# YaqiangCao/cLoops

Measured on AMD Instinct MI355X. Metric: PETs clustered/sec (whole node) + wall-clock for mode-3 eps x minPts sweep, higher is better.
Workload: dtype int32; 1 GPU; synthetic-200M-23chr-mode3 (BASELINE.json configs[3]); variant=cDBSCAN2, pets=200000000, chromosomes=23, chained_cut=True, final_cut=3871, candidate_loops=3651369, parallelism=23 chromosomes LPT-sharded over 1 GPU(s)

## Files before the change

cloops_amd/csrc/k_lists.hip:

```cpp
#include "cl_chrom.h"

#ifdef CLOOPS_DEVEL
#define L_ABL(bit) (g.dbg2 & (bit))
#else
#define L_ABL(bit) 0
#endif
#ifdef CLOOPS_DEVEL
__device__ unsigned long long g_lstat[32];
__device__ __forceinline__ void lstat_add(int slot, int v)
{
    int t = v;
    for (int o = 32; o > 0; o >>= 1) t += __shfl_down(t, o);
    if ((threadIdx.x & 63) == 0 && t) atomicAdd(&g_lstat[slot], (unsigned long long)t);
}
extern "C" void cl_debug_lstats(unsigned long long* out)
{
    (void)hipDeviceSynchronize();
    (void)hipMemcpyFromSymbol(out, HIP_SYMBOL(g_lstat), sizeof(g_lstat));
    unsigned long long z[32] = {0};
    (void)hipMemcpyToSymbol(HIP_SYMBOL(g_lstat), z, sizeof(z));
}
#define LSTAT_ON (g.dbg2 & (1 << 30))
#define LSTAT(slot, v) do { if (LSTAT_ON) lstat_add((slot), (v)); } while (0)
#else
// ... 476 lines not shown
        cgv[u] = cgloc[gidx]; wgv[u] = wgloc[gidx];
        const int b = t0 + u * 256 + (int)threadIdx.x;
        q[u] = b < npos ? bq[b] : 0; sp[u] = b < npos ? bsp[b] : 0;
    }
    {
        int2 fx[8];
#pragma unroll
        for (int u = 0; u < 8; ++u) {
            const int b = t0 + u * 256 + (int)threadIdx.x;
            const bool isc = (cbv[u] >> lane) & 1ull, isw = (wbv[u] >> lane) & 1ull;
            const int* wsrc = (BAND && q[u] < bandq) ? band : words;
            aux[u] = L_ABL(1 << 25) ? b : (isw ? wsrc[b] : (isc ? (V2 ? bkey[b] : (int)brow[b]) : 0));
            fx[u] = make_int2(INT_MIN, 0);
            if (V2 && CUT && !L_ABL(1 << 26)) {
                const unsigned long long anyb = cbv[u] | wbv[u];
                const int st = isc ? (sp[u] >> g.rbits) : 0;
                if (anyb) {
                    const int s_lo = __builtin_amdgcn_readlane(sp[u], __ffsll((long long)anyb) - 1) >> g.rbits;
                    const int s_hi = __builtin_amdgcn_readlane(sp[u], 63 - __clzll((long long)anyb)) >> g.rbits;
                    const int2 fa = fix[s_lo], fz = fix[s_hi];
                    if (isc) fx[u] = st == s_lo ? fa : (st == s_hi ? fz : fix[st]);
                }
            }
        }
#pragma unroll
        for (int u = 0; u < 8; ++u) {
            const int b = t0 + u * 256 + (int)threadIdx.x;
            const bool isw = (wbv[u] >> lane) & 1ull;
            if (V2 && CUT && b < fx[u].x) aux[u] = fx[u].y;
            if (isw) aux[u] = (int)lh_pack(aux[u], 0, 0);
        }
    }
    int cbase, wbase;
    {
        const int sb = blk >> 4;
        int pc = 0, pw_ = 0;
        for (int k = threadIdx.x; k < sb; k += 256) { const unsigned long long v = sup[k]; pc += (int)(unsigned)v; pw_ += (int)(unsigned)(v >> 32); }
        if (threadIdx.x < 16) { const int k = sb * 16 + (int)threadIdx.x; if (k < blk) { pc += bsum[k]; pw_ += bsum[nblk + 1 + k]; } }
#pragma unroll
        for (int o = 32; o > 0; o >>= 1) { pc += __shfl_down(pc, o); pw_ += __shfl_down(pw_, o); }
        if (lane == 0) { l_red[0][wv] = pc; l_red[1][wv] = pw_; }
        __syncthreads();
        cbase = l_red[0][0] + l_red[0][1] + l_red[0][2] + l_red[0][3];
        wbase = l_red[1][0] + l_red[1][1] + l_red[1][2] + l_red[1][3];
    }
    if (blk == nblk - 1 && threadIdx.x == 0) {
        const int C = cbase + bsum[blk], W = wbase + bsum[nblk + 1 + blk];
        lcnt[0] = C; lcnt[1] = W;
        cgrank[nblk * LG] = C; wgrank[nblk * LG] = W;
#ifdef CLOOPS_DEVEL
        if (LSTAT_ON) { atomicAdd(&g_lstat[8], (unsigned long long)C); atomicAdd(&g_lstat[9], (unsigned long long)W); atomicAdd(&g_lstat[11], 1ull); }
#endif
    }
#pragma unroll
    for (int u = 0; u < 8; ++u) {
        cgv[u] += cbase; wgv[u] += wbase;
        if (lane == 0) { const int gidx = (t0 >> 6) + u * 4 + wv; cgrank[gidx] = cgv[u]; wgrank[gidx] = wgv[u]; }
    }
#pragma unroll
    for (int u = 0; u < 8; ++u) {
        const int b = t0 + u * 256 + (int)threadIdx.x;
        const unsigned long long cb = cbv[u], wb = wbv[u];
        const bool isc = (cb >> lane) & 1ull, isw = (wb >> lane) & 1ull;
        if (L_ABL(1 << 27)) { if (q[u] + sp[u] + aux[u] == 0x7f123457) ckey[0] = 1; continue; }
        if (isc) {
            const int dst = cgv[u] + __popcll(cb & low_mask(lane));
            cpair[dst] = make_int2(q[u], sp[u]); ckey[dst] = aux[u];
            if (cpos) cpos[dst] = b;
            if (parent) parent[dst] = dst;
        } else if (isw) {
            const int dst = wgv[u] + __popcll(wb & low_mask(lane));
            wpair[dst] = make_int2(q[u], sp[u]); wpos[dst] = b; wenc[dst] = aux[u];
        }
    }
}

#define CH_PER 4
__global__ void __launch_bounds__(256)
k_chain_c(GridParams g, const int* __restrict__ lcnt, const int2* __restrict__ cpair, int* __restrict__ chainid,
          int* __restrict__ parent, int* __restrict__ compkey, int* __restrict__ ncore, int* __restrict__ bsize,
          int* __restrict__ usize, int* __restrict__ state, int* __restrict__ cskip,
          const int* __restrict__ strip_start, const unsigned long long* __restrict__ cmask, const int* __restrict__ cgrank,
          int* __restrict__ cstrip, int* __restrict__ sup, int nsup2, int* __restrict__ ckey_prune )
{
    const int C = lcnt[0];
    const int lane = threadIdx.x & 63;
    const int nmask = ~(g.peps - 1);
    {
        const int M = strip_start[g.S];
        for (int u = blockIdx.x * 256 + (int)threadIdx.x; u <= g.S + 1; u += gridDim.x * 256) {
            const int p = u <= g.S ? strip_start[u] : M;
            cstrip[u] = p < M ? core_rank(cmask, cgrank, p) : C;
        }
        if (blockIdx.x == 0) for (int k = threadIdx.x; k < nsup2; k += 256) sup[k] = 0;
    }
    int2 me[CH_PER], pv[CH_PER], nx[CH_PER];
#pragma unroll
    for (int e = 0; e < CH_PER; ++e) {
        const int c = (blockIdx.x * CH_PER + e) * 256 + (int)threadIdx.x;
        const bool in = c < C;
        me[e] = in ? cpair[c] : make_int2(0, 0);
        pv[e] = (in && c > 0) ? cpair[c - 1] : make_int2(0, INT_MIN);
        nx[e] = (in && c + 1 < C) ? cpair[c + 1] : make_int2(0, INT_MIN);
    }
#pragma unroll
    for (int e = 0; e < CH_PER; ++e) {
        const int c = (blockIdx.x * CH_PER + e) * 256 + (int)threadIdx.x;
        const bool in = c < C;
        const int p0 = me[e].y & nmask;
        const bool open = in && (c == 0 || (pv[e].y & nmask) != p0 || pv[e].x < me[e].x - g.eps);
        const bool last = in && (c + 1 >= C || (nx[e].y & nmask) != p0 || nx[e].x > me[e].x + g.eps);
        const unsigned long long ob = __ballot(open);
        const unsigned long long lb = __ballot(last) & (~0ull << lane);
        const int skip = (c - lane) + (lb ? __ffsll((long long)lb) : 64);
        const unsigned long long upto = ob & ((2ull << lane) - 1ull);
        int head = upto ? (c - lane) + 63 - __clzll((long long)upto) : -1;
        if (__any(in && !upto)) {
            int found = -1;
            for (int k0 = (c - lane) - 64; found < 0 && k0 >= 0; k0 -= 64) {
                const int j = k0 + lane;
                const int2 a = cpair[j];
                const int2 b = j > 0 ? cpair[j - 1] : make_int2(0, INT_MIN);
                const bool o = j == 0 || (b.y & nmask) != (a.y & nmask) || b.x < a.x - g.eps;
                const unsigned long long bal = __ballot(o);
                if (bal) found = k0 + 63 - __clzll((long long)bal);
            }
            if (!upto) head = found;
        }
        if (in) {
            chainid[c] = head;
            if (head == c) { parent[c] = c; compkey[c] = INT_MAX; ncore[c] = 0; bsize[c] = 0; usize[c] = 0; state[c] = ST_LIVE; }
            cskip[c] = skip;
            if (ckey_prune && c > 0 && (pv[e].y & nmask) == p0 && div_eps(g, pv[e].x) == div_eps(g, me[e].x)) ckey_prune[c] = INT_MAX;
        }
    }
}

#define LU_MAXB 4
__device__ __forceinline__ int lower_bound_pairs(const int2* __restrict__ pv, int lo, int hi, int val)
{
    while (hi - lo > 4) {
        const int qq = (hi - lo) >> 2;
        const int m1 = lo + qq, m2 = m1 + qq, m3 = m2 + qq;
        const int v1 = pv[m1].x, v2 = pv[m2].x, v3 = pv[m3].x;
        if (v1 >= val) hi = m1;
        else if (v2 >= val) { lo = m1 + 1; hi = m2; }
        else if (v3 >= val) { lo = m2 + 1; hi = m3; }
        else lo = m3 + 1;
    }
    while (lo < hi && pv[lo].x < val) ++lo;
    return lo;
}

struct HeadReset { int* compkey; int* ncore; int* bsize; int* usize; int* state; };
template <int NT, int HALO, bool FUSE>
__global__ void __launch_bounds__(256)
k_union_c(GridParams g, int ntiles, const int* __restrict__ lcnt, const int2* __restrict__ cpair, int* chainid,
          const int* __restrict__ cstrip, int* cskip, int* parent, HeadReset hr, int* __restrict__ ckey_prune ,
          int* __restrict__ ovlist, int* __restrict__ counters)
{
    constexpr int WIN = NT + HALO;
    constexpr int NCH = WIN / 64;
    __shared__ int2 lw[WIN];
    __shared__ int lx[WIN];
    __shared__ int lend[WIN];
    __shared__ unsigned long long l_ob[FUSE ? NCH : 1];
    __shared__ int l_found;
    const int C = lcnt[0];
    const int tile = ltile_of_block(blockIdx.x);
    const int t0 = tile * NT;
    if (tile >= ntiles || t0 >= C) return;
    const int base = t0 - HALO;
    const int lane = threadIdx.x & 63;
    const int nmask = ~(g.peps - 1);
    if (FUSE && threadIdx.x == 0) l_found = -1;
    int pf_tb[NT / 256], pf_b[NT / 256];
    {
        constexpr int SU = (WIN + 255) / 256;
        static_assert(WIN % 64 == 0, "whole waves in the last staging round");
        int2 mv[SU], pvl[SU];
#pragma unroll
        for (int u = 0; u < SU; ++u) {
            const int gi = base + u * 256 + (int)threadIdx.x;
            const bool in = gi >= 0 && gi < C && u * 256 + (int)threadIdx.x < WIN;
            mv[u] = in ? cpair[gi] : (gi < 0 ? make_int2(0, INT_MIN) : make_int2(INT_MAX, INT_MAX));
            pvl[u] = (FUSE && lane == 0 && gi > 0 && gi < C) ? cpair[gi - 1] : make_int2(0, 0);
        }
        if (HALO % 256 == 0) {
#pragma unroll
            for (int u2 = 0; u2 < NT / 256; ++u2) {
                const int gi = t0 + u2 * 256 + (int)threadIdx.x;
                const int s = mv[HALO / 256 + u2].y >> g.rbits;
                const bool ok = gi < C && s > 0;
                pf_tb[u2] = ok ? cstrip[s - 1] : 0; pf_b[u2] = ok ? cstrip[s] : 0;
            }
        }
#pragma unroll
        for (int u = 0; u < SU; ++u) {
            const int k = u * 256 + (int)threadIdx.x, gi = base + k;
            if (k >= WIN) continue;
            const bool in = gi >= 0 && gi < C;
            const int2 me = mv[u];
            lw[k] = me;
            if (!FUSE) { lx[k] = in ? chainid[gi] : -1; lend[k] = in ? cskip[gi] : 0; }
            else {
                int2 pv = make_int2(wave_shr1(me.x), wave_shr1(me.y));
                if (lane == 0 && gi > 0 && gi < C) pv = pvl[u];
                const bool o = gi <= 0 ? gi == 0 : (gi >= C || (pv.y & nmask) != (me.y & nmask) || pv.x < me.x - g.eps);
                const unsigned long long ob = __ballot(o);
                if (lane == 0) l_ob[k >> 6] = ob;
            }
        }
    }
    __syncthreads();
    if (FUSE) {
        if (threadIdx.x < 64 && base > 0 && !(l_ob[0] & 1ull)) {
            int found = -1;
            for (int k0 = base - 64; found < 0; k0 -= 64) {
                const int j = k0 + lane;
                bool o = false;
                if (j >= 0) {
                    const int2 a = cpair[j];
                    const int2 b = j > 0 ? cpair[j - 1] : make_int2(0, INT_MIN);
                    o = j == 0 || (b.y & nmask) != (a.y & nmask) || b.x < a.x - g.eps;
                }
                const unsigned long long bal = __ballot(o);
                if (bal) found = k0 + 63 - __clzll((long long)bal);
            }
            if (lane == 0) l_found = found;
        }
        __syncthreads();
        for (int k = threadIdx.x; k < WIN; k += 256) {
            const int ch = k >> 6, gi = base + k;
            const unsigned long long ob = l_ob[ch];
            const unsigned long long upto = ob & (~0ull >> (63 - lane));
            int head;
            if (upto) head = base + ch * 64 + 63 - __clzll((long long)upto);
            else {
                head = l_found;
                for (int c2 = ch - 1; c2 >= 0; --c2) { const unsigned long long o2 = l_ob[c2]; if (o2) { head = base + c2 * 64 + 63 - __clzll((long long)o2); break; } }
            }
            const unsigned long long above = lane == 63 ? 0ull : (ob & (~0ull << (lane + 1)));
            int skip;
            if (above) skip = base + ch * 64 + __ffsll((long long)above) - 1;
            else {
                skip = base + WIN;
                for (int c2 = ch + 1; c2 < NCH; ++c2) { const unsigned long long o2 = l_ob[c2]; if (o2) { skip = base + c2 * 64 + __ffsll((long long)o2) - 1; break; } }
            }
            const bool in = gi >= 0 && gi < C;
            lx[k] = in ? head : -1;
            lend[k] = in ? min(skip, C) : 0;
            if (in && k >= HALO) {
                chainid[gi] = head;
                cskip[gi] = min(skip, C);
                if (head == gi) { hr.compkey[gi] = INT_MAX; hr.ncore[gi] = 0; hr.bsize[gi] = 0; hr.usize[gi] = 0; hr.state[gi] = ST_LIVE; }
                if (ckey_prune && gi > 0) {
                    const int2 me = lw[k], pv = lw[k - 1];
                    if ((pv.y & nmask) == (me.y & nmask) && div_eps(g, pv.x) == div_eps(g, me.x)) ckey_prune[gi] = INT_MAX;
                }
            }
        }
        __syncthreads();
    }
    const int wbeg = max(base, 0);
    LdsPairs w; w.a = lw; w.base = base;
    constexpr int PER = NT / 256;
#pragma unroll 1
    for (int u = 0; u < PER; ++u) {
        const int i = t0 + u * 256 + (int)threadIdx.x;
        const bool in = i < C;
        int Bs[LU_MAXB];
#pragma unroll
        for (int k = 0; k < LU_MAXB; ++k) Bs[k] = -1;
        int nb = 0;
        int A = -1;
#ifdef CLOOPS_DEVEL
        int st_it = 0, st_touch = 0, st_glb = 0, st_jump = 0;
#endif
        if (in) {
            const int2 me = lw[i - base];
            A = lx[i - base];
            const int s = me.y >> g.rbits;
            int tb, b;
            if (HALO % 256 == 0) { tb = u == 0 ? pf_tb[0] : pf_tb[NT / 256 - 1]; b = u == 0 ? pf_b[0] : pf_b[NT / 256 - 1]; }
            else { tb = s > 0 ? cstrip[s - 1] : 0; b = s > 0 ? cstrip[s] : 0; }
            if (tb < b) {
                const int qlo = me.x - g.eps, qhi = me.x + g.eps;
                const int T = me.y - g.peps;
                if (tb < wbeg && wbeg < b && lw[wbeg - base].x < qlo) tb = wbeg;
                auto touch = [&](int B) {
                    bool seen = false;
#pragma unroll
                    for (int k = 0; k < LU_MAXB; ++k) seen |= (Bs[k] == B);
                    if (seen) return;
#ifdef CLOOPS_DEVEL
                    ++st_touch;
#endif
                    if (nb < LU_MAXB) {
#pragma unroll
                        for (int k = 0; k < LU_MAXB; ++k) if (k == nb) Bs[k] = B;
                        ++nb;
                    } else {
                        uf_unite(parent, A, B);
                    }
                };
                if (L_ABL(1 << 17)) tb = b;
                if (tb >= b) { }
                else if (tb >= wbeg && b - tb <= 2047) {
                    const int len = b - tb;
                    int j;
                    if (len <= 31) j = lds_lower_bound8<5>(w, tb, b, qlo);
                    else if (len <= 63) j = lds_lower_bound8<6>(w, tb, b, qlo);
                    else if (len <= 255) j = lds_lower_bound8<8>(w, tb, b, qlo);
                    else j = lds_lower_bound8<11>(w, tb, b, qlo);
                    if (L_ABL(1 << 16)) j = b;
                    while (j < b) {
#ifdef CLOOPS_DEVEL
                        ++st_it;
#endif
                        int2 cv[4];
#pragma unroll
                        for (int k = 0; k < 4; ++k) cv[k] = lw[min(j + k, b - 1) - base];
                        int f = 4; bool fh = false;
#pragma unroll
                        for (int k = 3; k >= 0; --k) {
                            const bool bey = (j + k >= b) | (cv[k].x > qhi);
                            const bool hit = cv[k].y >= T;
                            if (bey | hit) { f = k; fh = hit & !bey; }
                        }
                        if (f == 4) { j += 4; continue; }
                        if (!fh) break;
                        const int idx = j + f - base;
                        touch(lx[idx]);
#ifdef CLOOPS_DEVEL
                        ++st_jump;
#endif
                        j = lend[idx];
                    }
                } else if (FUSE) {
                    ovlist[atomicAdd(&counters[CTR_NOVF], 1)] = i;
                } else {
#ifdef CLOOPS_DEVEL
                    ++st_glb;
#endif
                    int k = lower_bound_pairs(cpair, tb, b, qlo);
                    while (k < b) {
                        int2 cv[4]; int bv[4];
#pragma unroll
                        for (int e = 0; e < 4; ++e) { const int idx = min(k + e, b - 1); cv[e] = cpair[idx]; bv[e] = chainid[idx]; }
                        int next = k + 4;
                        bool stop = false;
#pragma unroll
                        for (int e = 0; e < 4; ++e) {
                            if (stop || k + e >= b) continue;
                            if (cv[e].x > qhi) { stop = true; next = b; continue; }
                            if (cv[e].y >= T) {
                                touch(bv[e]);
                                stop = true;
                                next = cskip[min(k + e, b - 1)];
                            }
                        }
                        k = next;
                    }
                }
            }
        }
        int st_un = 0;
#pragma unroll
        for (int k = 0; k < LU_MAXB; ++k) {
            const int B = Bs[k];
            unsigned long long pending = __ballot(B >= 0);
            bool rep = false;
            while (pending) {
                const int leader = __ffsll((long long)pending) - 1;
                const int LA = __builtin_amdgcn_readlane(A, leader), LB = __builtin_amdgcn_readlane(B, leader);
                const unsigned long long m = __ballot(B >= 0 && A == LA && B == LB);
                if (lane == leader) rep = true;
                pending &= ~m;
            }
            if (rep && !L_ABL(1 << 15)) { uf_unite(parent, A, B); ++st_un; }
        }
#ifdef CLOOPS_DEVEL
        LSTAT(12, in ? 1 : 0); LSTAT(13, st_it); LSTAT(14, st_touch); LSTAT(15, st_un); LSTAT(16, st_glb); LSTAT(17, st_jump);
        { int mx = st_it; for (int o2 = 32; o2 > 0; o2 >>= 1) mx = max(mx, __shfl_down(mx, o2)); if (lane == 0 && LSTAT_ON) { atomicAdd(&g_lstat[18], (unsigned long long)mx); atomicAdd(&g_lstat[19], 1ull); }
          if (LSTAT_ON && st_it > 2) atomicAdd(&g_lstat[20], 1ull); if (LSTAT_ON && st_it > 4) atomicAdd(&g_lstat[21], 1ull); if (LSTAT_ON && st_it > 8) atomicAdd(&g_lstat[22], 1ull); }
#else
        (void)st_un;
#endif
    }
}

__global__ void k_prep_c(GridParams g, const int* __restrict__ lcnt, const int* __restrict__ strip_start,
                         const unsigned long long* __restrict__ cmask, const int* __restrict__ cgrank, int* __restrict__ cstrip,
                         int* __restrict__ sup, int nsup2, int* __restrict__ parent )
{
    const int C = lcnt[0];
    const int u = blockIdx.x * blockDim.x + threadIdx.x;
    if (parent && u < C) parent[u] = u;
    if (u <= g.S + 1) {
        const int M = strip_start[g.S];
        const int p = u <= g.S ? strip_start[u] : M;
        cstrip[u] = p < M ? core_rank(cmask, cgrank, p) : C;
    }
    if (u < nsup2) sup[u] = 0;
}
__global__ void k_union_overflow(GridParams g, const int* __restrict__ counters, const int* __restrict__ ovlist, const int2* __restrict__ cpair,
                                 const int* __restrict__ chainid, const int* __restrict__ cstrip, const int* __restrict__ cskip, int* parent)
{
    const int nov = counters[CTR_NOVF];
    for (int t = blockIdx.x * blockDim.x + threadIdx.x; t < nov; t += gridDim.x * blockDim.x) {
        const int i = ovlist[t];
        const int2 me = cpair[i];
        const int A = chainid[i];
        const int s = me.y >> g.rbits;
        if (s <= 0) continue;
        const int tb = cstrip[s - 1], b = cstrip[s];
        const int qlo = me.x - g.eps, qhi = me.x + g.eps, T = me.y - g.peps;
        int k = lower_bound_pairs(cpair, tb, b, qlo);
        int lastB = -1;
        while (k < b) {
            int2 cv[8];
#pragma unroll
            for (int e = 0; e < 8; ++e) cv[e] = cpair[min(k + e, b - 1)];
            int f = 8; bool fh = false;
#pragma unroll
            for (int e = 7; e >= 0; --e) {
                const bool bey = (k + e >= b) | (cv[e].x > qhi);
                const bool hit = cv[e].y >= T;
                if (bey | hit) { f = e; fh = hit & !bey; }
            }
            if (f == 8) { k += 8; continue; }
            if (!fh) break;
            const int B = chainid[k + f];
            if (B != lastB) { uf_unite(parent, A, B); lastB = B; }
            k = cskip[k + f];
        }
    }
}

#ifndef FLC_TPB
#define FLC_TPB BIGTPB
#endif
#ifndef FLC_PER
#define FLC_PER 4
#endif
__global__ void __launch_bounds__(FLC_TPB)
k_flatten_c(const int* __restrict__ lcnt, const int* __restrict__ chainid, const int* __restrict__ parent, const int* __restrict__ ckey,
            int* __restrict__ croot, int* __restrict__ compkey,
            int* __restrict__ ncore, int* __restrict__ rootlist, int* __restrict__ counters, int abl)
{
    __shared__ int hkey[AGG_H], hmin[AGG_H], hcnt[AGG_H];
    __shared__ int l_nroot, l_rootbase;
    for (int k = threadIdx.x; k < AGG_H; k += FLC_TPB) { hkey[k] = -1; hmin[k] = INT_MAX; hcnt[k] = 0; }
    if (threadIdx.x == 0) l_nroot = 0;
    __syncthreads();
    const int C = lcnt[0];
    if ((int)blockIdx.x * FLC_TPB * FLC_PER >= C) return;
    int ii[FLC_PER], r[FLC_PER], key[FLC_PER], x[FLC_PER];
    bool in[FLC_PER];
#pragma unroll
    for (int e = 0; e < FLC_PER; ++e) {
        ii[e] = (blockIdx.x * FLC_PER + e) * FLC_TPB + (int)threadIdx.x;
        in[e] = ii[e] < C;
        x[e] = in[e] ? chainid[ii[e]] : -1;
        key[e] = in[e] ? ckey[ii[e]] : INT_MAX;
    }
    {
        bool todo = false;
#pragma unroll
        for (int e = 0; e < FLC_PER; ++e) todo |= in[e];
        if (abl & (1 << 21)) todo = false;
        while (todo) {
            int p[FLC_PER];
#pragma unroll
            for (int e = 0; e < FLC_PER; ++e) p[e] = in[e] ? parent[x[e]] : -1;
            todo = false;
#pragma unroll
            for (int e = 0; e < FLC_PER; ++e) { todo |= in[e] && p[e] != x[e]; x[e] = in[e] ? p[e] : x[e]; }
        }
    }
#pragma unroll
    for (int e = 0; e < FLC_PER; ++e) {
        r[e] = in[e] ? x[e] : -1;
        if (in[e]) croot[ii[e]] = r[e];
    }
    const int lane = threadIdx.x & 63;
    int myslot[FLC_PER];
#pragma unroll
    for (int e = 0; e < FLC_PER; ++e) {
        myslot[e] = -1;
        const bool isroot = r[e] == ii[e] && r[e] >= 0;
        const unsigned long long rb = __ballot(isroot);
        if (rb) {
            int wbase = 0;
            if (lane == 0) wbase = atomicAdd(&l_nroot, __popcll(rb));
            wbase = __builtin_amdgcn_readfirstlane(wbase);
            if (isroot) myslot[e] = wbase + lane_rank(rb);
        }
    }
    if (!(abl & (1 << 20)))
#pragma unroll
    for (int e = 0; e < FLC_PER; ++e) {
        if (!__any(r[e] >= 0)) continue;
        const int rv = r[e];
        const WaveRuns w = wave_runs(rv);
        int mk = key[e];
        seg_step_min<0x111, 0xf>(w.dist >= 1, mk);
        seg_step_min<0x112, 0xf>(w.dist >= 2, mk);
        seg_step_min<0x114, 0xf>(w.dist >= 4, mk);
        seg_step_min<0x118, 0xf>(w.dist >= 8, mk);
        seg_step_min<0x142, 0xa>(w.dist > (lane & 15), mk);
        seg_step_min<0x143, 0xc>(w.dist > (lane & 31), mk);
        if (w.last && rv >= 0) {
            const int cntv = w.dist + 1;
            const int sl = agg_slot(hkey, rv);
            if (sl >= 0) { if (mk != INT_MAX) atomicMin(&hmin[sl], mk); atomicAdd(&hcnt[sl], cntv); }
            else { if (mk != INT_MAX) atomicMin(&compkey[rv], mk); atomicAdd(&ncore[rv], cntv); }
        }
    }
    __syncthreads();
    for (int k = threadIdx.x; k < AGG_H; k += FLC_TPB)
        if (hkey[k] >= 0) {
            atomicMin(&compkey[hkey[k]], hmin[k]);
            atomicAdd(&ncore[hkey[k]], hcnt[k]);
        }
    if (threadIdx.x == 0) l_rootbase = l_nroot ? atomicAdd(&counters[CTR_NROOT], l_nroot) : 0;
    __syncthreads();
#pragma unroll
    for (int e = 0; e < FLC_PER; ++e) if (myslot[e] >= 0) rootlist[l_rootbase + myslot[e]] = ii[e];
}

__global__ void k_scatter_by_pos(const int* __restrict__ cnt_ptr, const int* __restrict__ pos, const int* __restrict__ val, int* __restrict__ out)
{
    const int k = blockIdx.x * blockDim.x + threadIdx.x;
    if (k < cnt_ptr[0]) out[pos[k]] = val[k];
}
// ... 667 lines not shown
{
#define LA_ARGS g, (const int*)c->w_sv, (const int*)c->w_sa, (const int*)c->w_strip, c->ws, (const u32*)c->srow, b.cmask, b.wmask, b.hmask, b.cgloc, b.wgloc, b.bsum, b.sup, c->cellfirst.as<int>()
    if (g.variant == CL_VARIANT_CDBSCAN2) hipLaunchKernelGGL(k_classify<true>, dim3(nblk), dim3(256), 0, c->stream, LA_ARGS);
    else hipLaunchKernelGGL(k_classify<false>, dim3(nblk), dim3(256), 0, c->stream, LA_ARGS);
#undef LA_ARGS
}
static void launch_make_lists(cl_chrom* c, const GridParams& g, int nblk, const ListBufs& b, const ListRun& L)
{
#define LM_ARGS g, (const int*)c->w_sv, (const int*)c->w_sa, (const int*)c->w_strip, c->ws, (const u32*)c->srow, (const unsigned long long*)b.cmask,                   \
                (const unsigned long long*)b.wmask, (const unsigned long long*)b.hmask, (const int*)b.cgloc, (const int*)b.wgloc, (const int*)b.bsum, (const int*)b.sup,  \
                (const int*)c->cellfirst.as<int>(), b.cgrank, b.wgrank, L.cpair, L.cpos, L.ckey, L.wpair, L.wpos, L.wenc, b.lcnt
    if (g.variant == CL_VARIANT_CDBSCAN2) hipLaunchKernelGGL(k_make_lists<true>, dim3(nblk), dim3(256), 0, c->stream, LM_ARGS);
    else hipLaunchKernelGGL(k_make_lists<false>, dim3(nblk), dim3(256), 0, c->stream, LM_ARGS);
#undef LM_ARGS
}
static void list_views(cl_chrom* c, const ListBufs& b, ListRun* L)
{
    L->lcnt = b.lcnt; L->cmask = b.cmask; L->wmask = b.wmask; L->cgrank = b.cgrank; L->wgrank = b.wgrank;
    L->cpair = c->keys_in.as<int2>(); L->wpair = c->keys_out.as<int2>();
    L->cpos = c->head.as<int>(); L->ckey = c->hi.as<int>();
    L->wpos = c->l_wpos.as<int>(); L->wenc = c->l_wenc.as<int>(); L->cstrip = c->l_cstrip.as<int>();
}

static inline void fuse_knob(cl_chrom* c)
{
#ifdef CLOOPS_DEVEL
    const char* e = getenv("CLOOPS_FUSE");
    if (e) c->fuse_chains = atoi(e) != 0;
#else
    (void)c;
#endif
}

int lists_build(cl_chrom* c, const GridParams& g, int nm, ListRun* out)
{
    ListBufs b;
    int rc = list_bufs(c, g, nm, &b);
    if (rc) return rc;
    const int nblk = nblocks(nm, LT);
    ListRun L{};
    list_views(c, b, &L);
    if (c->l_sup_dirty) HIP_TRY(hipMemsetAsync(b.sup, 0, (size_t)b.nsup2 * 4, c->stream));
    c->l_sup_dirty = true;
    launch_classify(c, g, nblk, b);
    launch_make_lists(c, g, nblk, b, L);
    fuse_knob(c);
    if (c->fuse_chains)
        hipLaunchKernelGGL(k_prep_c, dim3(nblocks(std::max(std::max(nm, g.S + 2), b.nsup2))), dim3(TPB), 0, c->stream, g, (const int*)L.lcnt, (const int*)c->w_strip,
                           (const unsigned long long*)L.cmask, (const int*)L.cgrank, L.cstrip, b.sup, b.nsup2, c->parent.as<int>());
#ifdef CLOOPS_DEVEL
    else
    hipLaunchKernelGGL(k_chain_c, dim3(nblocks(nm, 256 * CH_PER)), dim3(256), 0, c->stream, g, L.lcnt, (const int2*)L.cpair, c->chainflag.as<int>(),
                       c->parent.as<int>(), c->compkey.as<int>(), c->ncore.as<int>(), c->bsize.as<int>(), c->usize.as<int>(), c->state.as<int>(),
                       c->cellfirst.as<int>() , (const int*)c->w_strip, L.cmask, L.cgrank, L.cstrip, b.sup, b.nsup2, (int*)nullptr);
#else
    { }
#endif
    L.npos = nm; L.pstrip = c->w_strip;
    *out = L;
    HIP_TRY(hipGetLastError());
    c->l_sup_dirty = false;
    return CL_OK;
}

int lists_base_keys(cl_chrom* c, const GridParams& g)
{
    const int n = (int)c->n;
    int rc = c->bkey.ensure((size_t)n * 4);
    if (rc) return rc;
    hipLaunchKernelGGL(k_base_keys, dim3(nblocks(n, LT)), dim3(256), 0, c->stream, g, n, (const int*)(c->bq.as<int>() + SORT_PAD),
                       (const int*)(c->bsp.as<int>() + SORT_PAD), (const u32*)c->brow.as<u32>(), c->bkey.as<int>());
    HIP_TRY(hipGetLastError());
    return CL_OK;
}

int lists_build_base(cl_chrom* c, const GridParams& g, int nm, ListRun* out)
{
    fuse_knob(c);
    const int n = (int)c->n;
    ListBufs b;
    int rc = list_bufs(c, g, n, &b);
    if (rc) return rc;
    const int nblk = nblocks(n, LT);
    const bool v2 = g.variant == CL_VARIANT_CDBSCAN2;
    ListRun L{};
    list_views(c, b, &L);
    L.npos = n; L.pstrip = c->bstrip.as<int>();
    unsigned long long* sup64 = (unsigned long long*)b.sup;
    const int nsup_ints = 2 * (nblk / 16 + 2);
    if (c->l_sup_dirty) HIP_TRY(hipMemsetAsync(b.sup, 0, (size_t)std::max(nsup_ints, b.nsup2) * 4, c->stream));
    c->l_sup_dirty = true;
    const int* bq = c->bq.as<int>() + SORT_PAD;
    const int* bsp = c->bsp.as<int>() + SORT_PAD;
    const u32* brow = c->brow.as<u32>();
    c->srow = c->brow.as<u32>();
    const int* words = c->rc_cnt.as<int>();
    const int* band = c->cnt.as<int>();
    const int thr = c->l4_cut ? g.cut - g.V0 : INT_MIN;
    const int bandq = c->ws.bandq;
#define LCQ_ARGS g, n, thr, bandq, bq, words, band, b.cmask, b.wmask, b.cgloc, b.wgloc, b.bsum, sup64
    if (!c->l4_cut) hipLaunchKernelGGL((k_classify_q<false, false>), dim3(nblk), dim3(256), 0, c->stream, LCQ_ARGS);
    else if (c->l4_band) hipLaunchKernelGGL((k_classify_q<true, true>), dim3(nblk), dim3(256), 0, c->stream, LCQ_ARGS);
    else hipLaunchKernelGGL((k_classify_q<true, false>), dim3(nblk), dim3(256), 0, c->stream, LCQ_ARGS);
#undef LCQ_ARGS
#define LMQ_ARGS g, n, bandq, bq, bsp, brow, (const int*)c->bkey.as<int>(), (const int2*)c->l_fix.as<int2>(), words, band, (const unsigned long long*)b.cmask,                  \
                 (const unsigned long long*)b.wmask, (const int*)b.cgloc, (const int*)b.wgloc, (const int*)b.bsum, (const unsigned long long*)sup64, b.cgrank, b.wgrank, L.cpair,  \
                 c->run_rows ? L.cpos : (int*)nullptr, L.ckey, L.wpair, L.wpos, L.wenc, b.lcnt, c->fuse_chains ? c->parent.as<int>() : (int*)nullptr
    if (v2) {
        if (!c->l4_cut) hipLaunchKernelGGL((k_make_lists_q<true, false, false>), dim3(nblk), dim3(256), 0, c->stream, LMQ_ARGS);
        else if (c->l4_band) hipLaunchKernelGGL((k_make_lists_q<true, true, true>), dim3(nblk), dim3(256), 0, c->stream, LMQ_ARGS);
        else hipLaunchKernelGGL((k_make_lists_q<true, true, false>), dim3(nblk), dim3(256), 0, c->stream, LMQ_ARGS);
    } else {
        if (c->l4_band) hipLaunchKernelGGL((k_make_lists_q<false, true, true>), dim3(nblk), dim3(256), 0, c->stream, LMQ_ARGS);
        else hipLaunchKernelGGL((k_make_lists_q<false, false, false>), dim3(nblk), dim3(256), 0, c->stream, LMQ_ARGS);
    }
#undef LMQ_ARGS
    fuse_knob(c);
    if (c->fuse_chains)
        hipLaunchKernelGGL(k_prep_c, dim3(nblocks(std::max(g.S + 2, std::max(nsup_ints, b.nsup2)))), dim3(TPB), 0, c->stream, g, (const int*)L.lcnt,
                           (const int*)L.pstrip, (const unsigned long long*)L.cmask, (const int*)L.cgrank, L.cstrip, b.sup, std::max(nsup_ints, b.nsup2), (int*)nullptr);
#ifdef CLOOPS_DEVEL
    else
    hipLaunchKernelGGL(k_chain_c, dim3(nblocks(nm, 256 * CH_PER)), dim3(256), 0, c->stream, g, L.lcnt, (const int2*)L.cpair, c->chainflag.as<int>(),
                       c->parent.as<int>(), c->compkey.as<int>(), c->ncore.as<int>(), c->bsize.as<int>(), c->usize.as<int>(), c->state.as<int>(),
                       c->cellfirst.as<int>() , L.pstrip, L.cmask, L.cgrank, L.cstrip, b.sup, std::max(nsup_ints, b.nsup2), v2 ? L.ckey : (int*)nullptr);
#else
    { }
#endif
    *out = L;
    HIP_TRY(hipGetLastError());
    c->l_sup_dirty = false;
    return CL_OK;
}

int lists_words_to_base(cl_chrom* c, const GridParams& g)
{
    const int n = (int)c->n;
    LAUNCH(k_words_to_base, n, g, n, (const int*)(c->bsp.as<int>() + SORT_PAD), (const int4*)c->l_tab.as<int4>(), (const int*)c->rc_poff.as<int>(),
           (const int*)c->cnt.as<int>(), c->rc_cnt.as<int>());
    HIP_TRY(hipGetLastError());
    return CL_OK;
}

static int* croot_of(cl_chrom* c) { return c->run_level >= 2 ? c->root.as<int>() : c->l_aux.as<int>(); }

int lists_union_flatten(cl_chrom* c, const GridParams& g, int nm, const ListRun& L)
{
    constexpr int UNT = 512;
    const int nt = nblocks(nm, UNT);
    const HeadReset hr{c->compkey.as<int>(), c->ncore.as<int>(), c->bsize.as<int>(), c->usize.as<int>(), c->state.as<int>()};
    int* prune = (c->run_level >= 4 && g.variant == CL_VARIANT_CDBSCAN2) ? L.ckey : (int*)nullptr;
#define LU_ARGS g, nt, L.lcnt, (const int2*)L.cpair, c->chainflag.as<int>(), (const int*)L.cstrip, c->cellfirst.as<int>() , \
                c->parent.as<int>(), hr, prune, c->ulist.as<int>() , c->counters.as<int>()
    if (c->fuse_chains) {
        if ((long long)c->n > 80LL * g.S) hipLaunchKernelGGL((k_union_c<UNT, 512, true>), dim3(ltile_grid(nt)), dim3(256), 0, c->stream, LU_ARGS);
        else hipLaunchKernelGGL((k_union_c<UNT, 128, true>), dim3(ltile_grid(nt)), dim3(256), 0, c->stream, LU_ARGS);
        hipLaunchKernelGGL(k_union_overflow, dim3(1024), dim3(256), 0, c->stream, g, (const int*)c->counters.as<int>(), (const int*)c->ulist.as<int>(), (const int2*)L.cpair,
                           (const int*)c->chainflag.as<int>(), (const int*)L.cstrip, (const int*)c->cellfirst.as<int>(), c->parent.as<int>());
    }
#ifdef CLOOPS_DEVEL
    else {
        if ((long long)c->n > 80LL * g.S) hipLaunchKernelGGL((k_union_c<UNT, 512, false>), dim3(ltile_grid(nt)), dim3(256), 0, c->stream, LU_ARGS);
        else hipLaunchKernelGGL((k_union_c<UNT, 128, false>), dim3(ltile_grid(nt)), dim3(256), 0, c->stream, LU_ARGS);
    }
#endif
#undef LU_ARGS
    hipLaunchKernelGGL(k_flatten_c, dim3(nblocks(nm, FLC_TPB * FLC_PER)), dim3(FLC_TPB), 0, c->stream, L.lcnt, (const int*)c->chainflag.as<int>(),
                       (const int*)c->parent.as<int>(), (const int*)L.ckey, croot_of(c),
                       c->compkey.as<int>(), c->ncore.as<int>(), c->rootlist.as<int>(), c->counters.as<int>(), (int)g.dbg2);
    HIP_TRY(hipGetLastError());
    return CL_OK;
}

int lists_scatter_root(cl_chrom* c, int nm, const ListRun& L)
{
    HIP_TRY(hipMemsetAsync(c->root.p, 0xFF, (size_t)nm * 4, c->stream));
    LAUNCH(k_scatter_by_pos, nm, L.lcnt, (const int*)L.cpos, (const int*)croot_of(c), c->root.as<int>());
    return CL_OK;
}

int lists_border(cl_chrom* c, const GridParams& g, int nm, const ListRun& L)
{
    constexpr int BNT = 2048, BHC = 256, BNQ = 1024, BHQ = 254;
    (void)nm;
    int kcap = 2, bqg = 16;
    bool queued = true;
#ifdef CLOOPS_DEVEL
    { const char* e = getenv("CLOOPS_BCAP"); if (e) kcap = atoi(e); queued = kcap > 0; e = getenv("CLOOPS_BQG"); if (e) bqg = atoi(e); }
#endif
    const int nt = nblocks(L.npos, (g.variant == CL_VARIANT_CDBSCAN1 || !queued) ? BNT : BNQ);
#define LB_ARGS g, nt, L.npos, L.lcnt, L.cmask, L.cgrank, L.wgrank, (const int2*)L.cpair, (const int*)croot_of(c), (const int*)c->cellfirst.as<int>(),    \
                (const int*)L.ckey, (const int*)L.cstrip, (const int2*)L.wpair, (const int*)L.wpos, (const int*)L.wenc, (const int*)c->compkey.as<int>(),                    \
                (const int*)c->ncore.as<int>(), c->owner.as<int>(), c->bsize.as<int>(), c->usize.as<int>(), c->chainflag.as<int>() ,  \
                c->counters.as<int>()
    if (g.variant == CL_VARIANT_CDBSCAN1) hipLaunchKernelGGL((k_border_w<BNT, BHC, true>), dim3(ltile_grid(nt)), dim3(256), 0, c->stream, LB_ARGS);
#ifdef CLOOPS_DEVEL
    else if (!queued) hipLaunchKernelGGL((k_border_w<BNT, BHC, false>), dim3(ltile_grid(nt)), dim3(256), 0, c->stream, LB_ARGS);
#endif
#define LBQ_ARGS g, nt, L.npos, kcap, L.lcnt, L.cmask, L.cgrank, L.wgrank, (const int2*)L.cpair, (const int*)croot_of(c), (const int*)c->cellfirst.as<int>(),           \
                 (const int*)L.cstrip, (const int2*)L.wpair, (const int*)L.wpos, (const int*)L.wenc, (const int*)c->compkey.as<int>(), (const int*)c->ncore.as<int>(),        \
                 c->owner.as<int>(), c->bsize.as<int>(), c->usize.as<int>(), c->chainflag.as<int>(), c->counters.as<int>()
#ifdef CLOOPS_DEVEL
    else if (bqg == 8) hipLaunchKernelGGL((k_border_q<BNQ, BHQ, 8>), dim3(ltile_grid(nt)), dim3(256), 0, c->stream, LBQ_ARGS);
    else if (bqg == 32) hipLaunchKernelGGL((k_border_q<BNQ, BHQ, 32>), dim3(ltile_grid(nt)), dim3(256), 0, c->stream, LBQ_ARGS);
#endif
    else hipLaunchKernelGGL((k_border_q<BNQ, BHQ, 16>), dim3(ltile_grid(nt)), dim3(256), 0, c->stream, LBQ_ARGS);
    (void)bqg;
#undef LBQ_ARGS
#undef LB_ARGS
    HIP_TRY(hipGetLastError());
    return CL_OK;
}

int lists_emit_records(cl_chrom* c, const GridParams& g, int nm, const ListRun& L)
{
    (void)nm;
    hipLaunchKernelGGL(k_emit_records_w, dim3(2048), dim3(TPB), 0, c->stream, g, L.lcnt, L.cmask, L.cgrank, (const int2*)L.cpair, (const int*)croot_of(c),
                       (const int*)L.cstrip, (const int2*)L.wpair, (const int*)L.wpos, (const int*)L.wenc, (const int*)c->compkey.as<int>(),
                       (const int*)c->state.as<int>(), (const int*)c->owner.as<int>(), c->recs.as<Rec>(), (int)c->n, c->counters.as<int>(),
                       (const int*)c->chainflag.as<int>());
    HIP_TRY(hipGetLastError());
    return CL_OK;
}

int lists_scatter_owner(cl_chrom* c, int nm, const ListRun& L)
{
    int* opos = c->l_aux.as<int>();
    HIP_TRY(hipMemsetAsync(opos, 0xFF, (size_t)nm * 4, c->stream));
    LAUNCH(k_scatter_by_pos, nm, L.lcnt, (const int*)L.cpos, (const int*)croot_of(c), opos);
    LAUNCH(k_scatter_by_pos, nm, L.lcnt + 1, (const int*)L.wpos, (const int*)c->owner.as<int>(), opos);
    return CL_OK;
}

int lists_final(cl_chrom* c, const GridParams& g, int nm, const ListRun& L, bool rows, int* pair_count)
{
    cl_chrom::Slot& sl = c->slot[c->cur];
    hipLaunchKernelGGL(k_final_lists, dim3(nblocks(nm, LF_TPB * LF_CHUNKS)), dim3(LF_TPB), 0, c->stream, g, L.lcnt, (const int2*)L.cpair, (const int*)L.cpos,
                       (const int*)croot_of(c), (const int2*)L.wpair, (const int*)L.wpos, (const int*)c->owner.as<int>(), (const int*)c->chainhead.as<int>(),
                       (const u32*)c->srow, (rows && !c->pairs_out) ? sl.labels.as<int>() : (int*)nullptr, sl.slab.as<int>(), c->l_dist.as<int>(), make_table(c),
                       c->pairs_out ? sl.pairs.as<int2>() : (int2*)nullptr, (int)std::min<long long>(c->pairs_cap, INT_MAX), pair_count);
    HIP_TRY(hipGetLastError());
    return CL_OK;
}

#define RM_T 2048
__global__ void __launch_bounds__(256)
k_rowmask_count(int n, const int* __restrict__ labels, unsigned long long* __restrict__ mask, int* __restrict__ tsum,
                unsigned long long* __restrict__ sup)
{
    __shared__ int l_c[4];
    const int t0 = (int)blockIdx.x * RM_T;
    const int lane = threadIdx.x & 63, wv = threadIdx.x >> 6;
    int lab[8];
#pragma unroll
    for (int u = 0; u < 8; ++u) { const int r = t0 + u * 256 + (int)threadIdx.x; lab[u] = r < n ? labels[r] : -1; }
    int cnt = 0;
#pragma unroll
    for (int u = 0; u < 8; ++u) {
        const unsigned long long bal = __ballot(lab[u] >= 0);
        if (lane == 0 && t0 + u * 256 + wv * 64 < n) mask[(t0 >> 6) + u * 4 + wv] = bal;
        cnt += __popcll(bal);
    }
    if (lane == 0) l_c[wv] = cnt;
    __syncthreads();
    if (threadIdx.x == 0) {
        const int tot = l_c[0] + l_c[1] + l_c[2] + l_c[3];
        tsum[blockIdx.x] = tot;
        if (tot) atomicAdd(&sup[blockIdx.x >> 4], (unsigned long long)tot);
    }
}
__global__ void __launch_bounds__(256)
k_rowmask_write(int n, const int* __restrict__ labels, const unsigned long long* __restrict__ mask, const int* __restrict__ tsum,
                const unsigned long long* __restrict__ sup, int* __restrict__ out, long long cap, int* __restrict__ total)
{
    __shared__ long long l_red[4];
    __shared__ int l_goff[RM_T / 64];
    const int blk = (int)blockIdx.x, t0 = blk * RM_T;
    const int lane = threadIdx.x & 63, wv = threadIdx.x >> 6;
    int lab[8];
#pragma unroll
    for (int u = 0; u < 8; ++u) { const int r = t0 + u * 256 + (int)threadIdx.x; lab[u] = r < n ? labels[r] : -1; }
    long long pc = 0;
    const int sb = blk >> 4;
    for (int k = threadIdx.x; k < sb; k += 256) pc += (long long)sup[k];
    if (threadIdx.x < 16) { const int k = sb * 16 + (int)threadIdx.x; if (k < blk) pc += tsum[k]; }
#pragma unroll
    for (int o = 32; o > 0; o >>= 1) pc += __shfl_down(pc, o);
    if (lane == 0) l_red[wv] = pc;
    if (threadIdx.x < 64) {
        const int k = lane & 31;
        const int gi = (t0 >> 6) + k;
        const int v = (lane < 32 && (long long)gi * 64 < n) ? __popcll(mask[gi]) : 0;
        int incl = v;
#pragma unroll
        for (int d = 1; d < 32; d <<= 1) { const int t = __shfl_up(incl, d, 32); incl += k >= d ? t : 0; }
        if (lane < 32) l_goff[k] = incl - v;
    }
    __syncthreads();
    const long long base = l_red[0] + l_red[1] + l_red[2] + l_red[3];
    if (blk == (int)gridDim.x - 1 && threadIdx.x == 0) *total = (int)(base + tsum[blk]);
#pragma unroll
    for (int u = 0; u < 8; ++u) {
        const unsigned long long bal = __ballot(lab[u] >= 0);
        if (lab[u] >= 0) {
            const long long dst = base + l_goff[u * 4 + wv] + __popcll(bal & low_mask(lane));
            if (dst < cap) out[dst] = lab[u];
        }
    }
}
int lists_rowmask(cl_chrom* c, int* total)
{
    cl_chrom::Slot& sl = c->slot[c->cur];
    const long long n = c->n;
    const size_t nw = (size_t)((n + 63) / 64), ntile = (size_t)((n + RM_T - 1) / RM_T), nsup = ntile / 16 + 1;
    const size_t cap = (size_t)std::max<long long>(c->mask_cap, 1);
    const size_t o_lab = nw * 8, o_tsum = ((o_lab + cap * 4 + 255) / 256) * 256, o_sup = ((o_tsum + ntile * 4 + 255) / 256) * 256;
    int rc = sl.pairs.ensure(o_sup + nsup * 8 + 256);
    if (rc) return rc;
// ... 88 lines not shown
```

Baseline: 14.90 billion PETs/s.

## Compact union work to cores not flanked by near neighbours; stage strip table in LDS

```diff
diff --git a/cloops_amd/csrc/k_lists.hip b/cloops_amd/csrc/k_lists.hip
--- a/cloops_amd/csrc/k_lists.hip
+++ b/cloops_amd/csrc/k_lists.hip
@@ -652,8 +652,9 @@
     return lo;
 }
 
+#define LU_STRIPS 64
 struct HeadReset { int* compkey; int* ncore; int* bsize; int* usize; int* state; };
-template <int NT, int HALO, bool FUSE>
+template <int NT, int HALO, bool FUSE, int UK>
 __global__ void __launch_bounds__(256)
 k_union_c(GridParams g, int ntiles, const int* __restrict__ lcnt, const int2* __restrict__ cpair, int* chainid,
           const int* __restrict__ cstrip, int* cskip, int* parent, HeadReset hr, int* __restrict__ ckey_prune ,
@@ -661,11 +662,16 @@
 {
     constexpr int WIN = NT + HALO;
     constexpr int NCH = WIN / 64;
+    constexpr int PER = NT / 256;
+    static_assert(NT % 256 == 0 && HALO % 64 == 0 && HALO >= UK && WIN <= 65536, "whole rounds of own cores, a wave-aligned halo that holds the test's reach, 16-bit work items");
     __shared__ int2 lw[WIN];
     __shared__ int lx[WIN];
     __shared__ int lend[WIN];
     __shared__ unsigned long long l_ob[FUSE ? NCH : 1];
     __shared__ int l_found;
+    __shared__ unsigned short l_work[NT];
+    __shared__ int l_nsurv[PER * 4];
+    __shared__ int l_cs[LU_STRIPS];
     const int C = lcnt[0];
     const int tile = ltile_of_block(blockIdx.x);
     const int t0 = tile * NT;
@@ -674,7 +680,8 @@
     const int lane = threadIdx.x & 63;
     const int nmask = ~(g.peps - 1);
     if (FUSE && threadIdx.x == 0) l_found = -1;
-    int pf_tb[NT / 256], pf_b[NT / 256];
+    int pf_cs = 0;
+    static_assert(LU_STRIPS == 64, "one staged row of the strip table per lane of a wave");
     {
         constexpr int SU = (WIN + 255) / 256;
         static_assert(WIN % 64 == 0, "whole waves in the last staging round");
@@ -686,14 +693,9 @@
             mv[u] = in ? cpair[gi] : (gi < 0 ? make_int2(0, INT_MIN) : make_int2(INT_MAX, INT_MAX));
             pvl[u] = (FUSE && lane == 0 && gi > 0 && gi < C) ? cpair[gi - 1] : make_int2(0, 0);
         }
-        if (HALO % 256 == 0) {
-#pragma unroll
-            for (int u2 = 0; u2 < NT / 256; ++u2) {
-                const int gi = t0 + u2 * 256 + (int)threadIdx.x;
-                const int s = mv[HALO / 256 + u2].y >> g.rbits;
-                const bool ok = gi < C && s > 0;
-                pf_tb[u2] = ok ? cstrip[s - 1] : 0; pf_b[u2] = ok ? cstrip[s] : 0;
-            }
+        if (((int)threadIdx.x >> 6) == (HALO % 256) / 64) {
+            const int r = (__builtin_amdgcn_readfirstlane(mv[HALO / 256].y) >> g.rbits) - 1 + lane;
+            pf_cs = (r >= 0 && r <= g.S + 1) ? cstrip[r] : 0;
         }
 #pragma unroll
         for (int u = 0; u < SU; ++u) {
@@ -764,11 +766,47 @@
     }
     const int wbeg = max(base, 0);
     LdsPairs w; w.a = lw; w.base = base;
-    constexpr int PER = NT / 256;
+    const int klo = max(0, -base), khi = min(WIN, C - base);
+    if (((int)threadIdx.x >> 6) == (HALO % 256) / 64) l_cs[lane] = pf_cs;
+    int myrank[PER];
+#pragma unroll
+    for (int u = 0; u < PER; ++u) {
+        const int k = HALO + u * 256 + (int)threadIdx.x;
+        const bool in = k < khi;
+        const int2 me = lw[k];
+        int2 nl[UK], nr[UK];
+#pragma unroll
+        for (int d = 0; d < UK; ++d) { nl[d] = lw[k - 1 - d]; nr[d] = lw[min(k + 1 + d, WIN - 1)]; }
+        bool dl = false, dr = false;
+#pragma unroll
+        for (int d = 0; d < UK; ++d) {
+            dl |= (k - 1 - d >= klo) & ((nl[d].y & nmask) == (me.y & nmask)) & (me.x - nl[d].x <= g.eps) & (nl[d].y <= me.y);
+            dr |= (k + 1 + d < khi) & ((nr[d].y & nmask) == (me.y & nmask)) & (nr[d].x - me.x <= g.eps) & (nr[d].y < me.y);
+        }
+        const bool surv = in && (!(dl && dr) || L_ABL(1 << 14));
+        const unsigned long long sb = __ballot(surv);
+        myrank[u] = surv ? lane_rank(sb) : -1;
+        if (lane == 0) l_nsurv[u * 4 + ((int)threadIdx.x >> 6)] = __popcll(sb);
+        LSTAT(12, in ? 1 : 0);
+    }
+    __syncthreads();
+    int nwork = 0;
+    {
+        int run = 0;
+#pragma unroll
+        for (int u = 0; u < PER; ++u) {
+            int mine = 0;
+#pragma unroll
+            for (int v = 0; v < 4; ++v) { if (v == ((int)threadIdx.x >> 6)) mine = run; run += l_nsurv[u * 4 + v]; }
+            if (myrank[u] >= 0) l_work[mine + myrank[u]] = (unsigned short)(HALO + u * 256 + (int)threadIdx.x);
+        }
+        nwork = run;
+    }
+    __syncthreads();
 #pragma unroll 1
-    for (int u = 0; u < PER; ++u) {
-        const int i = t0 + u * 256 + (int)threadIdx.x;
-        const bool in = i < C;
+    for (int t = (int)threadIdx.x & ~63; t < nwork; t += 256) {
+        const bool in = t + lane < nwork;
+        const int i = in ? base + (int)l_work[t + lane] : C;
         int Bs[LU_MAXB];
 #pragma unroll
         for (int k = 0; k < LU_MAXB; ++k) Bs[k] = -1;
@@ -781,9 +819,12 @@
             const int2 me = lw[i - base];
             A = lx[i - base];
             const int s = me.y >> g.rbits;
-            int tb, b;
-            if (HALO % 256 == 0) { tb = u == 0 ? pf_tb[0] : pf_tb[NT / 256 - 1]; b = u == 0 ? pf_b[0] : pf_b[NT / 256 - 1]; }
-            else { tb = s > 0 ? cstrip[s - 1] : 0; b = s > 0 ? cstrip[s] : 0; }
+            int tb = 0, b = 0;
+            if (s > 0) {
+                const int rel = s - (lw[HALO].y >> g.rbits);
+                if (rel + 1 < LU_STRIPS) { tb = l_cs[rel]; b = l_cs[rel + 1]; }
+                else { tb = cstrip[s - 1]; b = cstrip[s]; }
+            }
             if (tb < b) {
                 const int qlo = me.x - g.eps, qhi = me.x + g.eps;
                 const int T = me.y - g.peps;
@@ -881,7 +922,8 @@
             if (rep && !L_ABL(1 << 15)) { uf_unite(parent, A, B); ++st_un; }
         }
 #ifdef CLOOPS_DEVEL
-        LSTAT(12, in ? 1 : 0); LSTAT(13, st_it); LSTAT(14, st_touch); LSTAT(15, st_un); LSTAT(16, st_glb); LSTAT(17, st_jump);
+        LSTAT(23, in ? 1 : 0);
+        LSTAT(13, st_it); LSTAT(14, st_touch); LSTAT(15, st_un); LSTAT(16, st_glb); LSTAT(17, st_jump);
         { int mx = st_it; for (int o2 = 32; o2 > 0; o2 >>= 1) mx = max(mx, __shfl_down(mx, o2)); if (lane == 0 && LSTAT_ON) { atomicAdd(&g_lstat[18], (unsigned long long)mx); atomicAdd(&g_lstat[19], 1ull); }
           if (LSTAT_ON && st_it > 2) atomicAdd(&g_lstat[20], 1ull); if (LSTAT_ON && st_it > 4) atomicAdd(&g_lstat[21], 1ull); if (LSTAT_ON && st_it > 8) atomicAdd(&g_lstat[22], 1ull); }
 #else
@@ -1855,18 +1897,25 @@
     int* prune = (c->run_level >= 4 && g.variant == CL_VARIANT_CDBSCAN2) ? L.ckey : (int*)nullptr;
 #define LU_ARGS g, nt, L.lcnt, (const int2*)L.cpair, c->chainflag.as<int>(), (const int*)L.cstrip, c->cellfirst.as<int>() , \
                 c->parent.as<int>(), hr, prune, c->ulist.as<int>() , c->counters.as<int>()
+    constexpr int UK = 4;
+    const bool big = (long long)c->n > 80LL * g.S;
+#define LU_LAUNCH(HALO_, FUSE_, UK_) hipLaunchKernelGGL((k_union_c<UNT, HALO_, FUSE_, UK_>), dim3(ltile_grid(nt)), dim3(256), 0, c->stream, LU_ARGS)
+    bool wide = false;
+#ifdef CLOOPS_DEVEL
+    { const char* e = getenv("CLOOPS_UNION_K"); wide = e && atoi(e) == 8; }
+#endif
     if (c->fuse_chains) {
-        if ((long long)c->n > 80LL * g.S) hipLaunchKernelGGL((k_union_c<UNT, 512, true>), dim3(ltile_grid(nt)), dim3(256), 0, c->stream, LU_ARGS);
-        else hipLaunchKernelGGL((k_union_c<UNT, 128, true>), dim3(ltile_grid(nt)), dim3(256), 0, c->stream, LU_ARGS);
+        if (!wide) { if (big) LU_LAUNCH(512, true, UK); else LU_LAUNCH(128, true, UK); }
+#ifdef CLOOPS_DEVEL
+        else { if (big) LU_LAUNCH(512, true, 8); else LU_LAUNCH(128, true, 8); }
+#endif
         hipLaunchKernelGGL(k_union_overflow, dim3(1024), dim3(256), 0, c->stream, g, (const int*)c->counters.as<int>(), (const int*)c->ulist.as<int>(), (const int2*)L.cpair,
                            (const int*)c->chainflag.as<int>(), (const int*)L.cstrip, (const int*)c->cellfirst.as<int>(), c->parent.as<int>());
     }
 #ifdef CLOOPS_DEVEL
-    else {
-        if ((long long)c->n > 80LL * g.S) hipLaunchKernelGGL((k_union_c<UNT, 512, false>), dim3(ltile_grid(nt)), dim3(256), 0, c->stream, LU_ARGS);
-        else hipLaunchKernelGGL((k_union_c<UNT, 128, false>), dim3(ltile_grid(nt)), dim3(256), 0, c->stream, LU_ARGS);
-    }
-#endif
+    else { if (big) LU_LAUNCH(512, false, UK); else LU_LAUNCH(128, false, UK); }
+#endif
+#undef LU_LAUNCH
 #undef LU_ARGS
     hipLaunchKernelGGL(k_flatten_c, dim3(nblocks(nm, FLC_TPB * FLC_PER)), dim3(FLC_TPB), 0, c->stream, L.lcnt, (const int*)c->chainflag.as<int>(),
                        (const int*)c->parent.as<int>(), (const int*)L.ckey, croot_of(c),
```

After: 15.16 billion PETs/s, median of 6. +1.7%, better.
